# zwpku/colvars-finder

Measured on AMD Instinct MI355X. Metric: MD frames/sec through EigenFunctionTask train step, higher is better.
Workload: dtype f32; 1 GPU; BASELINE config 3: alanine-dipeptide-shaped EigenFunctionTask, generator mode, k=3, 22 atoms, align+position features d_r=66, nets [66,20,20,20,1], diag_coeff, Adam; frames_per_gpu=100000, batch_per_gpu=20000, global_batch=20000, parallelism=dp1 (frames sharded; all-reduce of batch sums + flat gradient)

## Files before the change

### colvars-finder_amd/csrc/ef16_back.hip

```cpp
#include "ef16_common.hpp"

namespace {

struct Back16Args {
  int k;
  int64_t B;
  int64_t n_tiles;
  int64_t T;
  const float* w_lag;
};

template <int H, int NH, bool MULTI, bool GEN>
__global__ __launch_bounds__(256, 4) void ef16_back_kernel(Back16Args args, cvf_mlp_desc mlp, const float* __restrict__ theta,
                                                            const float* __restrict__ packed, const float* __restrict__ w,
                                                            const float* __restrict__ feat, const float* __restrict__ y_tiled,
                                                            const float* __restrict__ q_tiled, const double* __restrict__ coef,
                                                            float* __restrict__ slab, int32_t* __restrict__ step,
                                                            const float* __restrict__ saved) {
  constexpr int RT = Hid<H>::RT, NG = Hid<H>::NG;
  constexpr int RTO = (H + 15) / 16;
  constexpr int CTH = (H + 1 + 15) / 16;
  constexpr int NT = 256, WPB = 4;
  constexpr bool TAIL4 = RTO == 2 && H % 16 >= 1 && H % 16 <= 4;
  constexpr int kRows = 2 * H + 2 * (H + 1) + 16;
  __shared__ __attribute__((aligned(16))) float IMG[kRows * kPitch];
  __shared__ float PART[4 * (H + 1)];
  extern __shared__ float GI[];
  float* SA1 = IMG;
  float* SA2 = SA1 + H * kPitch;
  float* SB1 = SA2 + H * kPitch;
  float* SB2 = SB1 + (H + 1) * kPitch;
  const int tid = threadIdx.x, lane = tid & 63;
  const int wave = __builtin_amdgcn_readfirstlane(tid >> 6);
  const int col = lane & 15, q = lane >> 4, row16 = col, r0 = 4 * q;
  const int fo = 16 * wave + col;
  const int rowf = 4 * col + q;
  const int net = blockIdx.y, k = args.k, D = mlp.dims[0];
  const int CT1 = (D + 1 + 15) / 16;
  const int c0 = 16 * (CT1 - 1), nfeat = D - c0, ncol = nfeat + 1;
  const bool strip = ncol <= 4;
  const int CTM = strip ? CT1 - 1 : CT1;
  const int gbase = mlp.w_off[net][0];
  const int gspan = mlp.b_off[net][NH] + 1 - gbase;
  float* out = slab + (int64_t)blockIdx.x * mlp.n_params + gbase;

  {
    static_assert((kRows * kPitch) % 4 == 0, "IMG is zeroed in 16-byte pieces");
    float4* img4 = reinterpret_cast<float4*>(IMG);
    for (int i = tid; i < kRows * kPitch / 4; i += NT) img4[i] = float4{0.0f, 0.0f, 0.0f, 0.0f};
  }
  if (MULTI)
    for (int i = tid; i < gspan; i += NT) GI[i] = 0.0f;
  lds_barrier();
  if (tid < 64) SB1[H * kPitch + tid] = 1.0f;

  const PackLayout L = pack_layout(H, NH, D);
  const URows pk = urows(packed + (int64_t)net * L.per_net, L.per_net, lane);
  float wl[RT][4];
  load_hid_const_u<H>(urows(theta + mlp.w_off[net][NH], H, q), wl);
  const double gS1n = coef[net], gEtn = coef[k + k * k + net];
  const double gS1ln = GEN ? 0.0 : coef[2 * k + k * k + net], gS2ln = GEN ? 0.0 : coef[3 * k + k * k + net];
  const float one[1] = {1.0f};

  const __amdgpu_buffer_rsrc_t out_rs = __builtin_amdgcn_make_buffer_rsrc(out, 0, gspan * 4, 0x00020000);
  auto emit_tile = [&](int l, int n_out, int n_in, int rt, int ct, const f32x4& acc) {
    const int wo = mlp.w_off[net][l] - gbase, bo = mlp.b_off[net][l] - gbase;
    const int i = 16 * ct + row16;
    int ob = 16 * rt + r0;
    asm volatile("" : "+v"(ob));
#pragma unroll
    for (int r = 0; r < 4; ++r) {
      const int o = ob + r;
      const bool isw = o < n_out && i < n_in, isb = o < n_out && i == n_in;
      const int idx = isw ? wo + o * n_in + i : bo + (o < n_out ? o : 0);
      const float av = acc[r];
      if (MULTI) {
        if (isw || isb) GI[idx] += av;
      } else {
        __builtin_amdgcn_raw_buffer_store_b32(__builtin_bit_cast(int, av), out_rs, (isw || isb) ? idx * 4 : 0x7ffffff0, 0, 0);
      }
    }
  };
  auto outer2 = [&](const float* A1, const float* B1, const float* A2, const float* B2, int rt, int ct) {
    f32x4 acc = {0.0f, 0.0f, 0.0f, 0.0f};
    acc = outer_half(A1, B1, rt, ct, lane, acc);
    if constexpr (GEN) acc = outer_half(A2, B2, rt, ct, lane, acc);
    return acc;
  };

  auto emit_entry = [&](bool live, int idx, float v) {
    if (MULTI) {
      if (live) GI[idx] += v;
    } else {
      __builtin_amdgcn_raw_buffer_store_b32(__builtin_bit_cast(int, v), out_rs, live ? idx * 4 : 0x7ffffff0, 0, 0);
    }
  };
  auto emit_last = [&]() {
    if (wave == WPB - 1) {
      int i = lane;
      asm volatile("" : "+v"(i));
      const bool live = i <= H;
      const float v = strip_total(PART + (live ? i : H), H + 1);
      emit_entry(live, i < H ? mlp.w_off[net][NH] - gbase + i : mlp.b_off[net][NH] - gbase, v);
    }
  };
  auto emit_strip = [&]() {
    if (strip && 64 * wave < 4 * H) {
      int e = tid;
      asm volatile("" : "+v"(e));
      const int o = e >> 2, c = e & 3;
      const bool live = o < H && c < ncol;
      const float v = strip_total(SB1 + (o < H ? e : 0), 4 * H);
      emit_entry(live, c < nfeat ? mlp.w_off[net][0] - gbase + o * D + c0 + c : mlp.b_off[net][0] - gbase + o, v);
    }
  };

  for (int64_t tile = blockIdx.x; tile < args.n_tiles; tile += gridDim.x) {
    CVF_STAMP(8);
    const bool lagged = !GEN && tile >= args.T;
    const int64_t t0 = lagged ? tile - args.T : tile;
    const int64_t frame = t0 * CVF_TILE + fo;
    const bool valid = frame < args.B;
    const float wraw = w[valid ? frame : args.B - 1];
    float yb[CVF_MAX_NETS];
#pragma unroll
    for (int j = 0; j < CVF_MAX_NETS; ++j) yb[j] = y_tiled[(t0 * k + (j < k ? j : k - 1)) * CVF_TILE + fo];
    float ylag = 0.0f, wlraw = 0.0f;
    if constexpr (!GEN) {
      ylag = y_tiled[((args.T + t0) * k + net) * CVF_TILE + fo];
      wlraw = args.w_lag[valid ? frame : args.B - 1];
    }
    const URows sv = urows(saved + (tile * k + net) * (int64_t)(kHand<NH>() * NG * 256) + wave * 64, kHand<NH>() * NG * 256 - wave * 64, lane);
    Vec<H, 1> h[NH], e[NH > 1 ? NH - 1 : 1], t[NH];
#pragma unroll
    for (int l = 0; l < NH; ++l) {
#pragma unroll
      for (int rt = 0; rt < RT; ++rt) h[l].v[rt][0] = f32x4{0.0f, 0.0f, 0.0f, 0.0f};
#pragma unroll
      for (int g = 0; g < NG; ++g) h[l].v[g >> 2][0][g & 3] = sv.ld((l * NG + g) * 256);
    }
    if constexpr (GEN) {
#pragma unroll
      for (int l = 0; l + 1 < NH; ++l) {
#pragma unroll
        for (int rt = 0; rt < RT; ++rt) e[l].v[rt][0] = f32x4{0.0f, 0.0f, 0.0f, 0.0f};
#pragma unroll
        for (int g = 0; g < NG; ++g) e[l].v[g >> 2][0][g & 3] = sv.ld(((NH + l) * NG + g) * 256);
      }
#pragma unroll
      for (int rt = 0; rt < RT; ++rt) t[0].v[rt][0] = f32x4{0.0f, 0.0f, 0.0f, 0.0f};
#pragma unroll
      for (int g = 0; g < NG; ++g) t[0].v[g >> 2][0][g & 3] = sv.ld(((2 * NH - 1) * NG + g) * 256);
    }
    HFrag<H> ffr[NH > 1 ? NH - 1 : 1];
    if constexpr (GEN) {
#pragma unroll
      for (int l = 1; l < NH; ++l) load_hfrag_u<H>(ffr[l - 1], pk, L.fh(l));
    }
    const float* f_tile = feat + tile * (int64_t)D * CVF_TILE;
    const float* q_tile = GEN ? q_tiled + (tile * k + net) * (int64_t)D * CVF_TILE : nullptr;
    const float wb = valid ? wraw : 0.0f;
    float alpha, gamma = 0.0f;
    float ynet = 0.0f;
#pragma unroll
    for (int j = 0; j < CVF_MAX_NETS; ++j)
      if (j == net) ynet = yb[j];
    if (GEN || !lagged) {
      double a = gS1n;
#pragma unroll
      for (int j = 0; j < CVF_MAX_NETS; ++j)
        if (j < k) a += (j == net ? 2.0 : 1.0) * coef[k + net * k + j] * (double)yb[j];
      alpha = (float)((double)wb * a);
      if constexpr (GEN) gamma = (float)(2.0 * (double)wb * gEtn);
      else alpha = (float)((double)wb * a - 2.0 * (double)wb * gEtn * ((double)ylag - (double)ynet));
    } else {
      const double wlg = valid ? (double)wlraw : 0.0;
      alpha = (float)(wlg * (gS1ln + 2.0 * gS2ln * (double)ylag) + 2.0 * (double)wb * gEtn * ((double)ylag - (double)ynet));
    }
    CVF_STAMP(9);
    if constexpr (GEN) {
#pragma unroll
      for (int rt = 0; rt < RT; ++rt)
#pragma unroll
        for (int r = 0; r < 4; ++r) t[0].v[rt][0][r] *= gamma;
#pragma unroll
      for (int l = 1; l < NH; ++l) {
        Vec<H, 1> td;
        tangent_of<H, 1>(td, h[l - 1], t[l - 1]);
        init_bias<H, 1>(t[l], nullptr, q);
        hidden_mul<H, 1>(t[l], ffr[l - 1], td);
      }
    }
    CVF_STAMP(11);
    {
      const float pick = strip_rows<H>([&](int rt, int r) {
        const float hv = h[NH - 1].v[rt][0][r];
        if constexpr (GEN) return fmaf(alpha, hv, (1.0f - hv * hv) * t[NH - 1].v[rt][0][r]);
        else return alpha * hv;
      }, col);
      const float sa = row_sumf16(alpha);
      if (col < NG && rowf < H) PART[wave * (H + 1) + rowf] = pick;
      if (lane == 0) PART[wave * (H + 1) + H] = sa;
    }
    CVF_STAMP(12);
    Vec<H, 1> hbar;
#pragma unroll
    for (int rt = 0; rt < RT; ++rt)
#pragma unroll
      for (int r = 0; r < 4; ++r) hbar.v[rt][0][r] = alpha * wl[rt][r];
    HFrag<H> tfl;
    float4 bA[4], bB[4];
    float xs[3] = {0.0f, 0.0f, 0.0f}, qs[3] = {0.0f, 0.0f, 0.0f};
    auto request = [&](float4 (&dst)[4], const float* src_tile, int ct) {
      const int i = 16 * ct + row16;
      const float4* p = reinterpret_cast<const float4*>(src_tile + (int64_t)(i < D ? i : D - 1) * CVF_TILE + 4 * q);
#pragma unroll
      for (int j = 0; j < 4; ++j) dst[j] = p[4 * j];
    };
    auto request_step = [&](int l) {
      if (l > 0) {
        load_hfrag_u<H>(tfl, pk, L.th(l));
      } else {
        if (strip) {
#pragma unroll
          for (int c = 0; c < 3; ++c)
            if (c < nfeat) {
              xs[c] = f_tile[(int64_t)(c0 + c) * CVF_TILE + fo];
              if constexpr (GEN) qs[c] = q_tile[(int64_t)(c0 + c) * CVF_TILE + fo];
            }
        }
        request(bA, f_tile, wave);
        if constexpr (GEN) request(bB, q_tile, wave);
      }
    };
    request_step(NH - 1);
#pragma unroll
    for (int l = NH - 1; l >= 0; --l) {
      CVF_STAMP(13 + (NH - 1 - l));
      Vec<H, 1> zbar, dl;
#pragma unroll
      for (int rt = 0; rt < RT; ++rt)
#pragma unroll
        for (int r = 0; r < 4; ++r) {
          const float hv = h[l].v[rt][0][r];
          const float om = 1.0f - hv * hv;
          if constexpr (GEN) {
            const float ev = (l == NH - 1) ? wl[rt][r] : e[l < NH - 1 ? l : 0].v[rt][0][r];
            const float hb = fmaf(-2.0f * hv * t[l].v[rt][0][r], ev, hbar.v[rt][0][r]);
            dl.v[rt][0][r] = ev * om;
            zbar.v[rt][0][r] = om * hb;
          } else {
            zbar.v[rt][0][r] = om * hbar.v[rt][0][r];
          }
        }
      store_image<H, 1, false>(SA1, zbar, one, lane, fo);
      if constexpr (GEN) {
        const float sc[1] = {l == 0 ? gamma : 1.0f};
        store_image<H, 1, true>(SA2, dl, sc, lane, fo);
      }
      if (l > 0) {
        store_image<H, 1, false>(SB1, h[l - 1], one, lane, fo);
        if constexpr (GEN) {
          Vec<H, 1> td;
          tangent_of<H, 1>(td, h[l - 1], t[l - 1]);
          store_image<H, 1, false>(SB2, td, one, lane, fo);
        }
        __syncthreads();
        init_bias<H, 1>(hbar, nullptr, q);
        hidden_mul<H, 1>(hbar, tfl, zbar);
        request_step(l - 1);
        if constexpr (TAIL4) {
          const int role = (wave + 2 * (l & 1)) & 3;
          if (role == 0) {
            emit_tile(l, H, H, 0, 0, outer2(SA1, SB1, SA2, SB2, 0, 0));
          } else {
            const int g = col >> 2, m = lane & 3;
            const int wo = mlp.w_off[net][l] - gbase, bo = mlp.b_off[net][l] - gbase;
            auto job = [&](int arow, int brow, int o, int i, bool live) {
              f32x4 acc = {0.0f, 0.0f, 0.0f, 0.0f};
              acc = outer_half44(SA1, arow, SB1, brow, lane, acc);
              if constexpr (GEN) acc = outer_half44(SA2, arow, SB2, brow, lane, acc);
              const float v = rows_sum_scatter(acc);
              asm volatile("" : "+v"(o));
              live = live && o < H && i <= H;
              emit_entry(live, i < H ? wo + o * H + i : bo + o, v);
            };
            const bool low = role == 1;
            const int cb = role == 3 ? 20 : 16;
            job(low ? 16 + m : 4 * g + m, low ? 4 * g + m : cb + m, low ? 16 + q : 4 * g + q, low ? 4 * g + m : cb + m, true);
            if (low) job(16 + m, 16 + 4 * (g & 1) + m, 16 + q, 16 + 4 * (g & 1) + m, g < 2);
          }
        } else {
          for (int pr = wave; pr < RTO * CTH; pr += WPB) {
            const int rt = pr / CTH, ct = pr - rt * CTH;
            emit_tile(l, H, H, rt, ct, outer2(SA1, SB1, SA2, SB2, rt, ct));
          }
        }
        if (l == NH - 1) emit_last();
        __syncthreads();
      } else {
        if (strip) {
#pragma unroll
          for (int c = 0; c < 4; ++c) {
            if (c < ncol) {
              const float xv = c == nfeat ? 1.0f : xs[c < 3 ? c : 2];
              const float qv = c == nfeat ? 0.0f : gamma * qs[c < 3 ? c : 2];
              const float pick = strip_rows<H>([&](int rt, int r) {
                if constexpr (GEN) return fmaf(zbar.v[rt][0][r], xv, dl.v[rt][0][r] * qv);
                else return zbar.v[rt][0][r] * xv;
              }, col);
              if (col < NG && rowf < H) SB1[(wave * H + rowf) * 4 + c] = pick;
            }
          }
        }
        __syncthreads();
        auto half0 = [&](f32x4 (&acc)[RTO], const float* SA, const float4 (&b)[4], int ct, int rt0, int rstep, bool ones) {
          const int i = 16 * ct + row16;
          const float pad = (ones && i == D) ? 1.0f : 0.0f;
#pragma unroll
          for (int rt = 0; rt < RTO; ++rt) {
            if (rt >= rt0 && (rt - rt0) % rstep == 0) {
              const float4* a1 = reinterpret_cast<const float4*>(SA + (16 * rt + row16) * kPitch + 4 * q);
              float4 av[4];
#pragma unroll
              for (int j = 0; j < 4; ++j) av[j] = a1[4 * j];
#pragma unroll
              for (int j = 0; j < 4; ++j) {
                acc[rt] = mfma4(av[j].x, i < D ? b[j].x : pad, acc[rt]);
                acc[rt] = mfma4(av[j].y, i < D ? b[j].y : pad, acc[rt]);
                acc[rt] = mfma4(av[j].z, i < D ? b[j].z : pad, acc[rt]);
                acc[rt] = mfma4(av[j].w, i < D ? b[j].w : pad, acc[rt]);
              }
            }
          }
        };
        const int extra = (CTM - WPB) * RTO;
        f32x4 acc[RTO];
#pragma unroll
        for (int rt = 0; rt < RTO; ++rt) acc[rt] = f32x4{0.0f, 0.0f, 0.0f, 0.0f};
        auto tail0 = [&](f32x4& tacc, const float* SA, const float4 (&b)[4], int ct, bool ones) {
          const int i = 16 * ct + row16;
          const float pad = (ones && i == D) ? 1.0f : 0.0f;
          const float4* a1 = reinterpret_cast<const float4*>(SA + (16 + (lane & 3)) * kPitch + 4 * q);
          float4 av[4];
#pragma unroll
          for (int j = 0; j < 4; ++j) av[j] = a1[4 * j];
#pragma unroll
          for (int j = 0; j < 4; ++j) {
            tacc = mfma1(av[j].x, i < D ? b[j].x : pad, tacc);
            tacc = mfma1(av[j].y, i < D ? b[j].y : pad, tacc);
            tacc = mfma1(av[j].z, i < D ? b[j].z : pad, tacc);
            tacc = mfma1(av[j].w, i < D ? b[j].w : pad, tacc);
          }
        };
        if (wave < CTM) {
          f32x4 tacc = {0.0f, 0.0f, 0.0f, 0.0f};
          half0(acc, SA1, bA, wave, 0, TAIL4 ? RTO : 1, true);
          if constexpr (TAIL4) tail0(tacc, SA1, bA, wave, true);
          if (wave < extra) request(bA, f_tile, WPB + wave / RTO);
          if constexpr (GEN) {
            half0(acc, SA2, bB, wave, 0, TAIL4 ? RTO : 1, false);
            if constexpr (TAIL4) tail0(tacc, SA2, bB, wave, false);
          }
#pragma unroll
          for (int rt = 0; rt < (TAIL4 ? 1 : RTO); ++rt) emit_tile(0, H, D, rt, wave, acc[rt]);
          if constexpr (TAIL4) {
            const float v = rows_sum_scatter(tacc);
            int o = 16 + q;
            asm volatile("" : "+v"(o));
            const int i = 16 * wave + row16;
            const bool isw = o < H && i < D, isb = o < H && i == D;
            emit_entry(isw || isb, isw ? mlp.w_off[net][0] - gbase + o * D + i : mlp.b_off[net][0] - gbase + (o < H ? o : 0), v);
          }
        }
        for (int pr = wave; pr < extra; pr += WPB) {
          const int ct = WPB + pr / RTO, rt = pr % RTO;
          if (pr != wave || wave >= CTM) request(bA, f_tile, ct);
          if constexpr (GEN) request(bB, q_tile, ct);
#pragma unroll
          for (int r_ = 0; r_ < RTO; ++r_) acc[r_] = f32x4{0.0f, 0.0f, 0.0f, 0.0f};
          half0(acc, SA1, bA, ct, rt, RTO, true);
          if constexpr (GEN) half0(acc, SA2, bB, ct, rt, RTO, false);
#pragma unroll
          for (int r_ = 0; r_ < RTO; ++r_)
            if (r_ == rt) emit_tile(0, H, D, r_, ct, acc[r_]);
        }
        emit_strip();
        if (NH == 1) emit_last();
        __syncthreads();
      }
    }
  }
  CVF_STAMP(17);
  if (MULTI) {
    __syncthreads();
    for (int i = tid; i < gspan; i += NT) out[i] = GI[i];
  }
  if (step != nullptr && blockIdx.x == 0 && blockIdx.y == 0 && tid == 0) *step += 1;
  CVF_STAMP(18);
}

}

extern "C" int64_t cvf_ef16_backward_slab_rows(int64_t n_tiles) { return n_tiles < 1024 ? n_tiles : 1024; }

static int ef16_backward_impl(const cvf_ef_cfg* cfg, const cvf_mlp_desc* mlp, const float* theta, const float* packed,
                              int64_t B, const float* w, const float* w_lag, const float* feat_tiled, const float* y_tiled,
                              const float* q_tiled, const double* coef, float* slab, int32_t* step_count, const float* saved,
                              void* stream) {
  const bool transfer = cfg != nullptr && cfg->lag_idx > 0;
  CVF_REQUIRE(cfg && mlp && theta && packed && w && feat_tiled && y_tiled && (transfer ? w_lag != nullptr : q_tiled != nullptr) && coef &&
              slab && saved && B > 0, "cvf_ef16_backward: bad argument");
  CVF_REQUIRE(cfg->k == mlp->n_nets, "cvf_ef16_backward: cfg.k must equal the number of nets");
  int H, NH;
  CVF_REQUIRE(ef16_shape(mlp, &H, &NH), "cvf_ef16_backward: unsupported net shape");
  CVF_REQUIRE(mlp->dims[0] <= 8 * 16 - 1, "cvf_ef16_backward: first layer wider than the column-tile schedule covers");
  const int span = mlp->b_off[0][NH] + 1 - mlp->w_off[0][0];
  int covered = 0;
  for (int n = 0; n < mlp->n_nets; ++n) {
    CVF_REQUIRE(mlp->b_off[n][NH] + 1 - mlp->w_off[n][0] == span, "cvf_ef16_backward: nets are not laid out contiguously");
    for (int l = 0; l <= NH; ++l)
      CVF_REQUIRE(mlp->w_off[n][l] >= mlp->w_off[n][0] && mlp->b_off[n][l] < mlp->w_off[n][0] + span,
                  "cvf_ef16_backward: nets are not laid out contiguously");
    covered += span;
  }
  CVF_REQUIRE(covered == mlp->n_params, "cvf_ef16_backward: flat buffer holds parameters outside the nets");
  Back16Args a;
  a.k = cfg->k;
  a.B = B;
  a.T = cvf_ntiles(B);
  a.n_tiles = transfer ? 2 * a.T : a.T;
  a.w_lag = w_lag;
  const int64_t G = cvf_ef16_backward_slab_rows(a.n_tiles);
  const bool launched = ef16_dispatch(H, NH, [&](auto h_, auto nh_) {
    constexpr int kH = decltype(h_)::value, kNH = decltype(nh_)::value;
    auto go = [&](auto kernel, size_t lds) {
      hipLaunchKernelGGL(kernel, dim3((unsigned)G, cfg->k), dim3(256), lds, (hipStream_t)stream, a, *mlp, theta, packed, w, feat_tiled,
                         y_tiled, q_tiled, coef, slab, step_count, saved);
    };
    const size_t gi = (size_t)span * sizeof(float);
    if (transfer) {
      if (a.n_tiles > G) go(ef16_back_kernel<kH, kNH, true, false>, gi);
      else go(ef16_back_kernel<kH, kNH, false, false>, 0);
    } else {
      if (a.n_tiles > G) go(ef16_back_kernel<kH, kNH, true, true>, gi);
      else go(ef16_back_kernel<kH, kNH, false, true>, 0);
    }
  });
  CVF_REQUIRE(launched, "cvf_ef16_backward: no kernel instance for hidden width %d x %d layers", H, NH);
  return cvf_check_launch("ef16_back_kernel");
}

extern "C" int cvf_ef16_backward(const cvf_ef_cfg* cfg, const cvf_mlp_desc* mlp, const float* theta, const float* packed,
                                 int64_t B, const float* w, const float* feat_tiled, const float* y_tiled, const float* q_tiled,
                                 const double* coef, float* slab, int32_t* step_count, const float* saved, void* stream) {
  CVF_REQUIRE(cfg && cfg->lag_idx == 0, "cvf_ef16_backward: generator mode (transfer-operator mode: cvf_ef16_backward_transfer)");
  return ef16_backward_impl(cfg, mlp, theta, packed, B, w, nullptr, feat_tiled, y_tiled, q_tiled, coef, slab, step_count, saved, stream);
}


extern "C" int cvf_ef16_backward_transfer(const cvf_ef_cfg* cfg, const cvf_mlp_desc* mlp, const float* theta, const float* packed,
                                          int64_t B, const float* w, const float* w_lag, const float* feat_tiled,
                                          const float* y_tiled, const double* coef, float* slab, int32_t* step_count,
                                          const float* saved, void* stream) {
  CVF_REQUIRE(cfg && cfg->lag_idx > 0, "cvf_ef16_backward_transfer: transfer-operator mode (cfg.lag_idx > 0)");
  return ef16_backward_impl(cfg, mlp, theta, packed, B, w, w_lag, feat_tiled, y_tiled, nullptr, coef, slab, step_count, saved, stream);
}
```

Before: 340.2 million frames/s.

## Compute per-net parameter offsets from template shape and hoist coefficient loads in backward kernel

```diff
diff --git a/colvars-finder_amd/csrc/ef16_back.hip b/colvars-finder_amd/csrc/ef16_back.hip
--- a/colvars-finder_amd/csrc/ef16_back.hip
+++ b/colvars-finder_amd/csrc/ef16_back.hip
@@ -9,9 +9,18 @@
   int64_t T;
   const float* w_lag;
 };
+struct Back16Nets {
+  int D;
+  int n_params;
+  int base[CVF_MAX_NETS];
+};
+template <int H, int NH>
+__host__ __device__ constexpr int net_w_off(int l, int hd) { return l == 0 ? 0 : hd + H + (l - 1) * (H * H + H); }
+template <int H, int NH>
+__host__ __device__ constexpr int net_b_off(int l, int hd) { return net_w_off<H, NH>(l, hd) + (l == 0 ? hd : l == NH ? H : H * H); }
 
 template <int H, int NH, bool MULTI, bool GEN>
-__global__ __launch_bounds__(256, 4) void ef16_back_kernel(Back16Args args, cvf_mlp_desc mlp, const float* __restrict__ theta,
+__global__ __launch_bounds__(256, 4) void ef16_back_kernel(Back16Args args, Back16Nets nets, const float* __restrict__ theta,
                                                             const float* __restrict__ packed, const float* __restrict__ w,
                                                             const float* __restrict__ feat, const float* __restrict__ y_tiled,
                                                             const float* __restrict__ q_tiled, const double* __restrict__ coef,
@@ -30,19 +39,33 @@
   float* SA2 = SA1 + H * kPitch;
   float* SB1 = SA2 + H * kPitch;
   float* SB2 = SB1 + (H + 1) * kPitch;
-  const int tid = threadIdx.x, lane = tid & 63;
+  const int tid = threadIdx.x;
   const int wave = __builtin_amdgcn_readfirstlane(tid >> 6);
-  const int col = lane & 15, q = lane >> 4, row16 = col, r0 = 4 * q;
-  const int fo = 16 * wave + col;
-  const int rowf = 4 * col + q;
-  const int net = blockIdx.y, k = args.k, D = mlp.dims[0];
-  const int CT1 = (D + 1 + 15) / 16;
-  const int c0 = 16 * (CT1 - 1), nfeat = D - c0, ncol = nfeat + 1;
-  const bool strip = ncol <= 4;
-  const int CTM = strip ? CT1 - 1 : CT1;
-  const int gbase = mlp.w_off[net][0];
-  const int gspan = mlp.b_off[net][NH] + 1 - gbase;
-  float* out = slab + (int64_t)blockIdx.x * mlp.n_params + gbase;
+  int lane = tid & 63, col, q, row16, r0, fo, rowf;
+  auto derive_lane = [&]() {
+    col = lane & 15, q = lane >> 4, row16 = col, r0 = 4 * q;
+    fo = 16 * wave + col;
+    rowf = 4 * col + q;
+  };
+  derive_lane();
+  static_assert(H % 4 == 0, "a lane's four rows of a gradient tile are inside the layer together (emit_tile)");
+  const int net = blockIdx.y;
+  int k = args.k;
+  int D = nets.D, HD, c0, nfeat, ncol, CTM;
+  bool strip;
+  PackLayout L;
+  auto derive = [&]() {
+    const int CT1 = (D + 1 + 15) / 16;
+    HD = H * D;
+    c0 = 16 * (CT1 - 1), nfeat = D - c0, ncol = nfeat + 1;
+    strip = ncol <= 4;
+    CTM = strip ? CT1 - 1 : CT1;
+    L = pack_layout(H, NH, D);
+  };
+  derive();
+  const int gbase = nets.base[net];
+  const int gspan = net_b_off<H, NH>(NH, HD) + 1;
+  float* out = slab + (int64_t)blockIdx.x * nets.n_params + gbase;
 
   {
     static_assert((kRows * kPitch) % 4 == 0, "IMG is zeroed in 16-byte pieces");
@@ -54,30 +77,28 @@
   lds_barrier();
   if (tid < 64) SB1[H * kPitch + tid] = 1.0f;
 
-  const PackLayout L = pack_layout(H, NH, D);
   const URows pk = urows(packed + (int64_t)net * L.per_net, L.per_net, lane);
   float wl[RT][4];
-  load_hid_const_u<H>(urows(theta + mlp.w_off[net][NH], H, q), wl);
-  const double gS1n = coef[net], gEtn = coef[k + k * k + net];
-  const double gS1ln = GEN ? 0.0 : coef[2 * k + k * k + net], gS2ln = GEN ? 0.0 : coef[3 * k + k * k + net];
+  load_hid_const_u<H>(urows(theta + gbase + net_w_off<H, NH>(NH, HD), H, q), wl);
   const float one[1] = {1.0f};
 
   const __amdgpu_buffer_rsrc_t out_rs = __builtin_amdgcn_make_buffer_rsrc(out, 0, gspan * 4, 0x00020000);
-  auto emit_tile = [&](int l, int n_out, int n_in, int rt, int ct, const f32x4& acc) {
-    const int wo = mlp.w_off[net][l] - gbase, bo = mlp.b_off[net][l] - gbase;
+  constexpr int kDead = 0x7fff0000;
+  auto emit_tile = [&](int l, int n_in, int rt, int ct, const f32x4& acc) {
+    const int wo = net_w_off<H, NH>(l, HD), bo = net_b_off<H, NH>(l, HD);
     const int i = 16 * ct + row16;
     int ob = 16 * rt + r0;
     asm volatile("" : "+v"(ob));
+    const bool isb = i == n_in, live = ob < H && i <= n_in;
+    const int idx0 = isb ? bo + ob : wo + ob * n_in + i, stride = isb ? 1 : n_in;
+    const int off0 = live ? idx0 * 4 : kDead;
 #pragma unroll
     for (int r = 0; r < 4; ++r) {
-      const int o = ob + r;
-      const bool isw = o < n_out && i < n_in, isb = o < n_out && i == n_in;
-      const int idx = isw ? wo + o * n_in + i : bo + (o < n_out ? o : 0);
       const float av = acc[r];
       if (MULTI) {
-        if (isw || isb) GI[idx] += av;
+        if (live) GI[idx0 + r * stride] += av;
       } else {
-        __builtin_amdgcn_raw_buffer_store_b32(__builtin_bit_cast(int, av), out_rs, (isw || isb) ? idx * 4 : 0x7ffffff0, 0, 0);
+        __builtin_amdgcn_raw_buffer_store_b32(__builtin_bit_cast(int, av), out_rs, off0 + r * stride * 4, 0, 0);
       }
     }
   };
@@ -92,7 +113,7 @@
     if (MULTI) {
       if (live) GI[idx] += v;
     } else {
-      __builtin_amdgcn_raw_buffer_store_b32(__builtin_bit_cast(int, v), out_rs, live ? idx * 4 : 0x7ffffff0, 0, 0);
+      __builtin_amdgcn_raw_buffer_store_b32(__builtin_bit_cast(int, v), out_rs, live ? idx * 4 : kDead, 0, 0);
     }
   };
   auto emit_last = [&]() {
@@ -101,7 +122,7 @@
       asm volatile("" : "+v"(i));
       const bool live = i <= H;
       const float v = strip_total(PART + (live ? i : H), H + 1);
-      emit_entry(live, i < H ? mlp.w_off[net][NH] - gbase + i : mlp.b_off[net][NH] - gbase, v);
+      emit_entry(live, i < H ? net_w_off<H, NH>(NH, HD) + i : net_b_off<H, NH>(NH, HD), v);
     }
   };
   auto emit_strip = [&]() {
@@ -111,12 +132,25 @@
       const int o = e >> 2, c = e & 3;
       const bool live = o < H && c < ncol;
       const float v = strip_total(SB1 + (o < H ? e : 0), 4 * H);
-      emit_entry(live, c < nfeat ? mlp.w_off[net][0] - gbase + o * D + c0 + c : mlp.b_off[net][0] - gbase + o, v);
-    }
-  };
-
-  for (int64_t tile = blockIdx.x; tile < args.n_tiles; tile += gridDim.x) {
+      emit_entry(live, c < nfeat ? o * D + c0 + c : HD + o, v);
+    }
+  };
+
+  int64_t tile = blockIdx.x;
+  do {
+    if constexpr (MULTI) {
+      asm volatile("" : "+s"(D), "+s"(k));
+      derive();
+      asm volatile("" : "+v"(lane));
+      derive_lane();
+    }
     CVF_STAMP(8);
+    double crow[CVF_MAX_NETS];
+#pragma unroll
+    for (int j = 0; j < CVF_MAX_NETS; ++j) crow[j] = coef[k + net * k + (j < k ? j : k - 1)];
+    double gS1n = coef[net], gEtn = coef[k + k * k + net];
+    double gS1ln = GEN ? 0.0 : coef[2 * k + k * k + net], gS2ln = GEN ? 0.0 : coef[3 * k + k * k + net];
+    __builtin_amdgcn_sched_barrier(0);
     const bool lagged = !GEN && tile >= args.T;
     const int64_t t0 = lagged ? tile - args.T : tile;
     const int64_t frame = t0 * CVF_TILE + fo;
@@ -165,11 +199,15 @@
 #pragma unroll
     for (int j = 0; j < CVF_MAX_NETS; ++j)
       if (j == net) ynet = yb[j];
+#pragma unroll
+    for (int j = 0; j < CVF_MAX_NETS; ++j) asm volatile("" : "+s"(crow[j]));
+    asm volatile("" : "+s"(gS1n), "+s"(gEtn));
+    if constexpr (!GEN) asm volatile("" : "+s"(gS1ln), "+s"(gS2ln));
     if (GEN || !lagged) {
       double a = gS1n;
 #pragma unroll
       for (int j = 0; j < CVF_MAX_NETS; ++j)
-        if (j < k) a += (j == net ? 2.0 : 1.0) * coef[k + net * k + j] * (double)yb[j];
+        if (j < k) a += (j == net ? 2.0 : 1.0) * crow[j] * (double)yb[j];
       alpha = (float)((double)wb * a);
       if constexpr (GEN) gamma = (float)(2.0 * (double)wb * gEtn);
       else alpha = (float)((double)wb * a - 2.0 * (double)wb * gEtn * ((double)ylag - (double)ynet));
@@ -272,10 +310,10 @@
         if constexpr (TAIL4) {
           const int role = (wave + 2 * (l & 1)) & 3;
           if (role == 0) {
-            emit_tile(l, H, H, 0, 0, outer2(SA1, SB1, SA2, SB2, 0, 0));
+            emit_tile(l, H, 0, 0, outer2(SA1, SB1, SA2, SB2, 0, 0));
           } else {
             const int g = col >> 2, m = lane & 3;
-            const int wo = mlp.w_off[net][l] - gbase, bo = mlp.b_off[net][l] - gbase;
+            const int wo = net_w_off<H, NH>(l, HD), bo = net_b_off<H, NH>(l, HD);
             auto job = [&](int arow, int brow, int o, int i, bool live) {
               f32x4 acc = {0.0f, 0.0f, 0.0f, 0.0f};
               acc = outer_half44(SA1, arow, SB1, brow, lane, acc);
@@ -293,7 +331,7 @@
         } else {
           for (int pr = wave; pr < RTO * CTH; pr += WPB) {
             const int rt = pr / CTH, ct = pr - rt * CTH;
-            emit_tile(l, H, H, rt, ct, outer2(SA1, SB1, SA2, SB2, rt, ct));
+            emit_tile(l, H, rt, ct, outer2(SA1, SB1, SA2, SB2, rt, ct));
           }
         }
         if (l == NH - 1) emit_last();
@@ -363,14 +401,14 @@
             if constexpr (TAIL4) tail0(tacc, SA2, bB, wave, false);
           }
 #pragma unroll
-          for (int rt = 0; rt < (TAIL4 ? 1 : RTO); ++rt) emit_tile(0, H, D, rt, wave, acc[rt]);
+          for (int rt = 0; rt < (TAIL4 ? 1 : RTO); ++rt) emit_tile(0, D, rt, wave, acc[rt]);
           if constexpr (TAIL4) {
             const float v = rows_sum_scatter(tacc);
             int o = 16 + q;
             asm volatile("" : "+v"(o));
             const int i = 16 * wave + row16;
             const bool isw = o < H && i < D, isb = o < H && i == D;
-            emit_entry(isw || isb, isw ? mlp.w_off[net][0] - gbase + o * D + i : mlp.b_off[net][0] - gbase + (o < H ? o : 0), v);
+            emit_entry(isw || isb, isw ? o * D + i : HD + (o < H ? o : 0), v);
           }
         }
         for (int pr = wave; pr < extra; pr += WPB) {
@@ -383,14 +421,15 @@
           if constexpr (GEN) half0(acc, SA2, bB, ct, rt, RTO, false);
 #pragma unroll
           for (int r_ = 0; r_ < RTO; ++r_)
-            if (r_ == rt) emit_tile(0, H, D, r_, ct, acc[r_]);
+            if (r_ == rt) emit_tile(0, D, r_, ct, acc[r_]);
         }
         emit_strip();
         if (NH == 1) emit_last();
         __syncthreads();
       }
     }
-  }
+    tile += gridDim.x;
+  } while (MULTI && tile < args.n_tiles);
   CVF_STAMP(17);
   if (MULTI) {
     __syncthreads();
@@ -425,6 +464,17 @@
     covered += span;
   }
   CVF_REQUIRE(covered == mlp->n_params, "cvf_ef16_backward: flat buffer holds parameters outside the nets");
+  for (int n = 0; n < mlp->n_nets; ++n)
+    for (int l = 0; l <= NH; ++l) {
+      CVF_REQUIRE(mlp->b_off[n][l] == mlp->w_off[n][l] + mlp->dims[l] * mlp->dims[l + 1],
+                  "cvf_ef16_backward: net %d, layer %d: the bias does not follow the weight", n, l);
+      CVF_REQUIRE(l == NH || mlp->w_off[n][l + 1] == mlp->b_off[n][l] + mlp->dims[l + 1],
+                  "cvf_ef16_backward: net %d: layer %d does not follow layer %d", n, l + 1, l);
+    }
+  Back16Nets nets;
+  nets.D = mlp->dims[0];
+  nets.n_params = mlp->n_params;
+  for (int n = 0; n < CVF_MAX_NETS; ++n) nets.base[n] = n < mlp->n_nets ? mlp->w_off[n][0] : 0;
   Back16Args a;
   a.k = cfg->k;
   a.B = B;
@@ -435,7 +485,7 @@
   const bool launched = ef16_dispatch(H, NH, [&](auto h_, auto nh_) {
     constexpr int kH = decltype(h_)::value, kNH = decltype(nh_)::value;
     auto go = [&](auto kernel, size_t lds) {
-      hipLaunchKernelGGL(kernel, dim3((unsigned)G, cfg->k), dim3(256), lds, (hipStream_t)stream, a, *mlp, theta, packed, w, feat_tiled,
+      hipLaunchKernelGGL(kernel, dim3((unsigned)G, cfg->k), dim3(256), lds, (hipStream_t)stream, a, nets, theta, packed, w, feat_tiled,
                          y_tiled, q_tiled, coef, slab, step_count, saved);
     };
     const size_t gi = (size_t)span * sizeof(float);
```

New measurement: 353.8 million frames/s, median of 6. 4.0% higher.
